# wdmwhh/MRefSR

Hardware: AMD Instinct MI355X
Metric: 4x SR Mpix/sec, 5-ref 160x160->640x640; PSNR within 0.01 dB of ref (higher is better)
Workload: dtype f32

## Files before the change

include/mrefsr_hip.h:

```cpp
#ifndef MREFSR_HIP_H
#define MREFSR_HIP_H

#include <stdint.h>

#ifdef __cplusplus
extern "C" {
#endif

#define MREFSR_ABI_VERSION 1

enum {
    MREFSR_OK = 0,
    MREFSR_E_INVALID = -1,
    MREFSR_E_UNSUPPORTED = -2,
    MREFSR_E_LAUNCH = -3
};

typedef void *mrefsr_stream_t;

int mrefsr_abi_version(void);
const char *mrefsr_last_error(void);


int mrefsr_corr_padded_channels(int C);
// ... 71 lines not shown
int mrefsr_conv_wgrad1x1_f32(const float *g, const float *x, const float *g_amax, float *grad_weight, void *workspace,
                             int64_t workspace_bytes, int64_t pixels, int Cout, int ld_g, int Cin, int ld_x, int *range_flag,
                             mrefsr_stream_t stream);
int mrefsr_dcn_fwd(const void *x, const void *offset, const void *mask, const void *weight, const void *bias,
                   void *out, const mrefsr_dcn_shape *s, float act_slope, int dtype, mrefsr_stream_t stream);
int mrefsr_dcn_im2col(const void *x, const void *offset, const void *mask, void *columns,
                      const mrefsr_dcn_shape *s, int dtype, mrefsr_stream_t stream);
int mrefsr_dcn_col2im(const void *grad_col, const void *x, const void *offset, const void *mask, void *grad_x,
                      void *grad_offset, void *grad_mask, const mrefsr_dcn_shape *s, int dtype,
                      mrefsr_stream_t stream);


int mrefsr_mrattn_fwd_f32(const float *q, const float *emb, const float *ass, float *out,
                          float *prob, int N, int T, int c, int c2, int HW, int t_major,
                          mrefsr_stream_t stream);
int mrefsr_mrattn_fwd_nhwc_f32(const float *q, const float *emb, const float *ass, float *out, int N,
                               int T, int c, int HW, mrefsr_stream_t stream);
int mrefsr_mrattn_fwd_nhwc_scaled_f32(const float *q, const float *emb, const float *ass, float *out, int N,
                                      int T, int c, int HW, float q_scale, mrefsr_stream_t stream);
int mrefsr_mrattn_bwd_f32(const float *q, const float *emb, const float *ass, const float *prob,
                          const float *g_out, float *g_q, float *g_emb, float *g_ass, int N,
                          int T, int c, int c2, int HW, int t_major, mrefsr_stream_t stream);
int mrefsr_mrattn_fwd_nhwc_bf16(const void *q, const void *emb, const void *ass, void *out, int N, int T,
                                int c, int HW, mrefsr_stream_t stream);
int mrefsr_mrattn_fwd_masked_f32(const float *q, const float *emb, const float *ass, const uint32_t *valid_bits, float *out,
                                 float *prob, int N, int T, int c, int c2, int HW, int t_major, mrefsr_stream_t stream);
int mrefsr_mrattn_bwd_masked_f32(const float *q, const float *emb, const float *ass, const float *prob, const float *g_out,
                                 const uint32_t *valid_bits, float *g_q, float *g_emb, float *g_ass, int N, int T, int c, int c2,
                                 int HW, int t_major, mrefsr_stream_t stream);
int mrefsr_mrattn_fwd_nhwc_masked_f32(const float *q, const float *emb, const float *ass, const uint32_t *valid_bits, float *out,
                                      int N, int T, int c, int HW, float q_scale, mrefsr_stream_t stream);
int mrefsr_mrattn_fwd_nhwc_masked_bf16(const void *q, const void *emb, const void *ass, const uint32_t *valid_bits, void *out, int N,
                                       int T, int c, int HW, mrefsr_stream_t stream);


int mrefsr_fused_bias_act(const void *x, const void *bias, const void *ref, void *out,
                          int64_t size_x, int step_b, int size_b, int act, int grad, float alpha,
                          float scale, int dtype, mrefsr_stream_t stream);

int mrefsr_tail_bilinear_add_f32(const float *y_nhwc, const float *x, float *out, int B, int C, int h, int w, int scale, int ld,
                                 mrefsr_stream_t stream);

int mrefsr_bias_act_res_f32(const float *x, const float *bias, const float *pre, int64_t pre_N,
                            const float *residual, float *out, int64_t N, int C, int64_t HW,
                            float slope, mrefsr_stream_t stream);

typedef struct mrefsr_conv_desc {
    int32_t N, H, W, ksize;
    int32_t C1, ld1, N1;
    int32_t C2, ld2, N2;
    int32_t Cout, ld_out, ld_res, pre_N;
    int32_t act, epilogue, terms;
    float slope;
    float wscale;
} mrefsr_conv_desc;
int64_t mrefsr_conv_packed_bytes(int Cout, int Cin, int ksize, int terms);
int mrefsr_conv_pack_weight_f32(const float *weight, void *packed, int Cout, int Cin, int ksize, int terms,
                                float wscale, mrefsr_stream_t stream);
int mrefsr_conv_pack_weight_view_f32(const float *weight, void *packed, int Cout, int Cin, int ksize, int terms, float wscale,
                                     int64_t stride_o, int64_t stride_i, int flip, mrefsr_stream_t stream);
typedef struct mrefsr_conv_pack_job {
    const float *weight;
    void *packed;
    int64_t stride_o, stride_i;
    int32_t Cout, Cin, ksize, terms, flip;
    float wscale;
// ... 328 lines not shown
```

mrefsr_amd/_lib.py:

```python
import ctypes as C
import os

_HERE = os.path.dirname(os.path.abspath(__file__))
LIB_PATH = os.environ.get('MREFSR_HIP_LIB') or os.path.join(_HERE, 'lib', 'libmrefsr_hip.so')
ABI_VERSION = 1

_vp, _i, _f, _i64 = C.c_void_p, C.c_int, C.c_float, C.c_int64


class DcnShape(C.Structure):
    _fields_ = [(n, C.c_int) for n in ('B', 'C', 'H', 'W', 'Co', 'kh', 'kw', 'stride_h', 'stride_w', 'pad_h', 'pad_w',
                                       'dil_h', 'dil_w', 'groups', 'dg')]


class ConvDesc(C.Structure):
    _fields_ = [(n, C.c_int32) for n in ('N', 'H', 'W', 'ksize', 'C1', 'ld1', 'N1', 'C2', 'ld2', 'N2', 'Cout', 'ld_out', 'ld_res',
                                         'pre_N', 'act', 'epilogue', 'terms')] + [('slope', C.c_float), ('wscale', C.c_float)]


class ConvPackJob(C.Structure):
    _fields_ = [('weight', C.c_void_p), ('packed', C.c_void_p), ('stride_o', C.c_int64), ('stride_i', C.c_int64), ('Cout', C.c_int32),
                ('Cin', C.c_int32), ('ksize', C.c_int32), ('terms', C.c_int32), ('flip', C.c_int32), ('wscale', C.c_float)]


# ... 26 lines not shown
    'mrefsr_pixnorm_f32': (_i, [_vp, _vp, _vp, _vp, _i, _i, _i, _i, _i, _i, _vp, _vp]),
    'mrefsr_patch_norm_f32': (_i, [_vp, _vp, _vp, _i, _i, _i, _vp]),
    'mrefsr_corr_top1_f32': (_i, [_vp, _vp, _vp, _vp, _vp, _vp, _i, _i, _i, _i, _i, _vp]),
    'mrefsr_feature_match_index_workspace_bytes': (_i64, [_i, _i, _i, _i]),
    'mrefsr_feature_match_index_f32': (_i, [_vp, _vp] + [_i] * 10 + [_vp, _vp, _vp, _i64, _vp]),
    'mrefsr_corr_workspace_bytes': (_i64, [_i, _i, _i]),
    'mrefsr_corr_prefilter_info': (_i64, [_i, _i, _i, _i, C.c_char_p, _i, C.POINTER(C.c_int)]),
    'mrefsr_corr_top1_prefilter_f32': (_i, [_vp] * 9 + [_i64, _i, _i, _i, _i, _i, _i, _vp, _vp]),
    'mrefsr_offsets_from_idx_f32': (_i, [_vp, _vp, _vp, _vp, _i, _i, _i, _vp]),
    'mrefsr_dynagg_prep_f32': (_i, [_vp, _vp, _vp, _vp, _vp, _vp, _i, _i, _i, _i, _i, _vp]),
    'mrefsr_dynagg_prep_bwd_f32': (_i, [_vp, _vp, _vp, _vp, _i, _i, _i, _i, _vp]),
    'mrefsr_dynagg_prep_bwd_nhwc_f32': (_i, [_vp, _vp, _vp, _vp, _vp, _vp, _i, _i, _i, _i, _vp]),
    'mrefsr_dynagg_prep_bwd_blocks': (_i, [_i, _i, _i, _i]),
    'mrefsr_dynagg_prep_bwd_det_workspace_bytes': (_i64, [_i, _i, _i, _i]),
    'mrefsr_dynagg_prep_bwd_nhwc_det_f32': (_i, [_vp, _vp, _vp, _vp, _vp, _vp, _i, _i, _i, _i, _vp, _i64, _vp, _vp]),
    'mrefsr_dcn_fwd_workspace_bytes': (_i64, [C.POINTER(DcnShape)]),
    'mrefsr_dcn_fwd_f32': (_i, [_vp, _vp, _vp, _vp, _vp, _vp, C.POINTER(DcnShape), _f, _i, _vp, _i64, _vp, _vp]),
    'mrefsr_dcn_fwd_amax_f32': (_i, [_vp, _vp, _vp, _vp, _vp, _vp, C.POINTER(DcnShape), _f, _i, _vp, _i64, _vp, _vp, _vp]),
    'mrefsr_dcn_im2col_f32': (_i, [_vp, _vp, _vp, _vp, C.POINTER(DcnShape), _vp]),
    'mrefsr_dcn_col2im_f32': (_i, [_vp, _vp, _vp, _vp, _vp, _vp, _vp, C.POINTER(DcnShape), _vp]),
    'mrefsr_dcn_bwd_data_f32': (_i, [_vp, _vp, _vp, _vp, _vp, _f, _vp, _vp, _vp, _vp, C.POINTER(DcnShape), _vp]),
    'mrefsr_dcn_bwd_weight_workspace_bytes': (_i64, [C.POINTER(DcnShape)]),
    'mrefsr_conv_wgrad1x1_workspace_bytes': (_i64, [_i64, _i, _i]),
    'mrefsr_conv_wgrad1x1_f32': (_i, [_vp, _vp, _vp, _vp, _vp, _i64, _i64, _i, _i, _i, _i, _vp, _vp]),
    'mrefsr_dcn_bwd_weight_f32': (_i, [_vp, _vp, _vp, _vp, _vp, _vp, _vp, _i64, C.POINTER(DcnShape), _vp, _vp]),
    'mrefsr_mrattn_fwd_f32': (_i, [_vp, _vp, _vp, _vp, _vp, _i, _i, _i, _i, _i, _i, _vp]),
    'mrefsr_mrattn_fwd_nhwc_f32': (_i, [_vp, _vp, _vp, _vp, _i, _i, _i, _i, _vp]),
    'mrefsr_mrattn_fwd_nhwc_scaled_f32': (_i, [_vp, _vp, _vp, _vp, _i, _i, _i, _i, _f, _vp]),
    'mrefsr_mrattn_bwd_f32': (_i, [_vp, _vp, _vp, _vp, _vp, _vp, _vp, _vp, _i, _i, _i, _i, _i, _i, _vp]),
    'mrefsr_mrattn_fwd_masked_f32': (_i, [_vp] * 6 + [_i] * 6 + [_vp]),
    'mrefsr_mrattn_bwd_masked_f32': (_i, [_vp] * 9 + [_i] * 6 + [_vp]),
    'mrefsr_mrattn_fwd_nhwc_masked_f32': (_i, [_vp] * 5 + [_i, _i, _i, _i, _f, _vp]),
    'mrefsr_mrattn_fwd_nhwc_masked_bf16': (_i, [_vp] * 5 + [_i, _i, _i, _i, _vp]),
    'mrefsr_fused_bias_act': (_i, [_vp, _vp, _vp, _vp, _i64, _i, _i, _i, _i, _f, _f, _i, _vp]),
    'mrefsr_bias_act_res_f32': (_i, [_vp, _vp, _vp, _i64, _vp, _vp, _i64, _i, _i64, _f, _vp]),
    'mrefsr_tail_bilinear_add_f32': (_i, [_vp, _vp, _vp, _i, _i, _i, _i, _i, _i, _vp]),
    'mrefsr_conv_packed_bytes': (_i64, [_i, _i, _i, _i]),
    'mrefsr_conv_pack_weight_f32': (_i, [_vp, _vp, _i, _i, _i, _i, _f, _vp]),
    'mrefsr_conv_pack_weight_view_f32': (_i, [_vp, _vp, _i, _i, _i, _i, _f, _i64, _i64, _i, _vp]),
    'mrefsr_conv_pack_weights_multi_f32': (_i, [_vp, _i, _vp, _vp]),
    'mrefsr_act_bwd_blocks': (_i, [_i64, _i]),
    'mrefsr_act_bwd_nhwc_f32': (_i, [_vp, _vp, _vp, _i, _vp, _vp, _vp, _i64, _i, _i, _f, _vp, _vp, _vp]),
    'mrefsr_act_bwd_det_workspace_bytes': (_i64, [_i64, _i]),
    'mrefsr_act_bwd_nhwc_det_f32': (_i, [_vp, _vp, _vp, _i, _vp, _vp, _vp, _i64, _i, _i, _f, _vp, _vp, _vp, _i64, _vp, _vp]),
    'mrefsr_conv_nhwc_scaled_f32': (_i, [C.POINTER(ConvDesc), _vp, _vp, _vp, _vp, _vp, _vp, _vp, _vp, _vp, _vp, _vp]),
    'mrefsr_conv_nhwc_amax_f32': (_i, [C.POINTER(ConvDesc), _vp, _vp, _vp, _vp, _vp, _vp, _vp, _vp, _vp, _vp, _vp, _vp]),
    'mrefsr_conv_nhwc_bwd_f32': (_i, [C.POINTER(ConvDesc), _vp, _vp, _vp, _i, _vp, _vp, _vp, _vp, _vp, _vp]),
    'mrefsr_conv_nhwc_bwd_det_workspace_bytes': (_i64, [C.POINTER(ConvDesc)]),
    'mrefsr_conv_nhwc_bwd_det_f32': (_i, [C.POINTER(ConvDesc), _vp, _vp, _vp, _i, _vp, _vp, _vp, _vp, _vp, _vp, _i64, _vp, _vp]),
    'mrefsr_conv_wgrad3x3_workspace_bytes': (_i64, [_i, _i, _i, _i, _i]),
    'mrefsr_conv_wgrad3x3_f32': (_i, [_vp, _i, _i, _vp, _i, _i, _vp, _i64, _i64, _i, _vp, _i, _i, _i, _vp, _i64, _vp, _vp]),
    'mrefsr_conv_wgrad3x3_batch_workspace_bytes': (_i64, [_i, _i, _i, _i, _i, _i]),
    'mrefsr_conv_wgrad3x3_batch_f32': (_i, [_i, _vp, _i, _i, _vp, _i, _i, _vp, _i64, _i64, _i, _vp, _i, _i, _i, _vp, _i64, _vp, _vp]),
    'mrefsr_mrattn_bwd_nhwc_f32': (_i, [_vp, _vp, _vp, _vp, _vp, _vp, _vp, _i, _i, _i, _i, _vp]),
    'mrefsr_mrattn_bwd_nhwc_masked_f32': (_i, [_vp] * 8 + [_i, _i, _i, _i, _vp]),
    'mrefsr_attn_modulate_bwd_f32': (_i, [_vp, _vp, _vp, _vp, _vp, _i64, _vp]),
    'mrefsr_reflect_pad_nhwc_f32': (_i, [_vp, _vp] + [_i] * 6 + [_vp]),
    'mrefsr_reflect_pad_bwd_nhwc_f32': (_i, [_vp, _vp] + [_i] * 6 + [_vp]),
    'mrefsr_crop_nhwc_f32': (_i, [_vp, _vp, _vp] + [_i] * 6 + [_vp]),
    'mrefsr_crop_bwd_nhwc_f32': (_i, [_vp, _vp] + [_i] * 6 + [_vp]),
    'mrefsr_conv_nhwc_f32': (_i, [C.POINTER(ConvDesc), _vp, _vp, _vp, _vp, _vp, _vp, _vp, _vp, _vp, _vp]),
    'mrefsr_dcn_fwd': (_i, [_vp, _vp, _vp, _vp, _vp, _vp, C.POINTER(DcnShape), _f, _i, _vp]),
    'mrefsr_dcn_im2col': (_i, [_vp, _vp, _vp, _vp, C.POINTER(DcnShape), _i, _vp]),
    'mrefsr_dcn_col2im': (_i, [_vp, _vp, _vp, _vp, _vp, _vp, _vp, C.POINTER(DcnShape), _i, _vp]),
    'mrefsr_conv_dynagg_f32': (_i, [C.POINTER(ConvDesc), _vp, _vp, _vp, _vp, _vp, _vp, _vp, _i, _vp, _vp]),
    'mrefsr_mrattn_fwd_nhwc_bf16': (_i, [_vp, _vp, _vp, _vp, _i, _i, _i, _i, _vp]),
# ... 180 lines not shown
```

mrefsr_amd/archs/ref_mrapa_restoration_arch.py:

```python
import logging

import torch
import torch.nn as nn
import torch.nn.functional as F
from torch.autograd import Function
from torch.autograd.function import once_differentiable

from .. import hip
from ..ops.dcn import modulated_deform_conv
from ..utils.registry import ARCH_REGISTRY
from . import nhwc, nhwc_train
from .arch_util import ResidualBlockNoBN, conv_act, default_init_weights, make_layer, ref_valid_bits, srntt_init_weights


class _DynAggPrep(Function):

    @staticmethod
    def forward(ctx, om, pre_offset, dg, abs_sum, om_bias=None):
        om = om.contiguous()
        offset, mask = hip.dynagg_prep(om, pre_offset.contiguous(), dg, abs_sum, om_bias)
        ctx.dg = dg
        ctx.save_for_backward(mask)
        return offset, mask

# ... 296 lines not shown
        return all((4 - s % 4) % 4 < s for side in (h, w) for s in (side, 2 * side))

    def spatial_padding(self, feats):
        _, _, h, w = feats.size()
        pad_h, pad_w = self.pads(h, w)
        if pad_h == 0 and pad_w == 0:
            return feats
        return F.pad(feats, [0, pad_w, 0, pad_h], mode='reflect')

    def forward(self, target, refs, ref_valid=None):
        t = len(refs)
        return self._fuse(target, torch.stack(refs, dim=1).flatten(0, 1), t, t_major=False, ref_valid=ref_valid)

    def forward_stacked(self, target, refs, t, ref_valid=None):
        return self._fuse(target, refs, t, t_major=True, ref_valid=ref_valid)

    def forward_nhwc(self, target, refs, t, ref_valid=None):
        h_in, w_in = target.shape[1:3]
        ph, pw = self.pads(h_in, w_in)
        vb = ref_valid_bits(ref_valid, target.shape[0], t, target.device)
        if ph or pw:
            if target.dtype != torch.float32:
                target = nhwc.to_nhwc(self.spatial_padding(nhwc.as_nchw(target)))
                refs = nhwc.to_nhwc(self.spatial_padding(nhwc.as_nchw(refs)))
                return self.forward_nhwc(target, refs, t, vb)[:, :h_in, :w_in, :].contiguous()
            out = self.forward_nhwc(nhwc.reflect_pad(target, ph, pw), nhwc.reflect_pad(refs, ph, pw), t, vb)
            return nhwc.crop(out, h_in, w_in)
        q = nhwc.conv(self.conv_emb1[0], target, prelu=self.conv_emb1[1], amax=False)
        train = q.requires_grad
        fold = not train and q.dtype == torch.float32 and not nhwc.BF16
        if not fold:
            q = q * self.scale if train else nhwc.rnd_(q.mul_(self.scale))
        emb = nhwc.conv(self.conv_emb2[0], refs, prelu=self.conv_emb2[1], amax=False)
        ass = nhwc.conv(self.conv_ass, refs, amax=False)
        if vb is not None:
            if fold:
                r = hip.mrattn_fwd_nhwc_masked(q, emb, ass, t, vb, q_scale=float(self.scale))
            else:
                r = nhwc_train.attention(q, emb, ass, t, vb) if train else nhwc.rnd_(hip.mrattn_fwd_nhwc_masked(q, emb, ass, t, vb))
        elif fold:
            r = hip.mrattn_fwd_nhwc(q, emb, ass, t, q_scale=float(self.scale))
        else:
            r = nhwc_train.attention(q, emb, ass, t) if train else nhwc.rnd_(hip.mrattn_fwd_nhwc(q, emb, ass, t))
        del emb, ass
        attn = nhwc.conv(self.spatial_attn, target, x2=r, slope=0.1)
        attn_mul = nhwc.conv(self.spatial_attn_mul2, nhwc.conv(self.spatial_attn_mul1, attn, slope=0.1), amax=False)
        attn_add = nhwc.conv(self.spatial_attn_add2, nhwc.conv(self.spatial_attn_add1, attn, slope=0.1), amax=False)
        r = nhwc_train.modulate(r, attn_mul, attn_add) if train else nhwc.rnd_(hip.attn_modulate_(r, attn_mul, attn_add))
        return nhwc.conv(self.feat_fusion, target, x2=r, slope=0.1)

    def _fuse(self, target, refs, t, t_major, ref_valid=None):
        h_input, w_input = target.shape[-2:]
        vb = ref_valid_bits(ref_valid, target.shape[0], t, target.device)
        target = self.spatial_padding(target)
        refs = self.spatial_padding(refs)
        q = self.conv_emb1(target) * self.scale
        emb = self.conv_emb2(refs)
        ass = conv_act(self.conv_ass, refs)
        refs = _MultiRefAttention.apply(q, emb, ass, t, t_major) if vb is None else _MultiRefAttention.apply(q, emb, ass, t, t_major, vb)
        attn = conv_act(self.spatial_attn, torch.cat([target, refs], dim=1), 0.1)
        attn_mul = conv_act(self.spatial_attn_mul2, conv_act(self.spatial_attn_mul1, attn, 0.1))
        attn_add = conv_act(self.spatial_attn_add2, conv_act(self.spatial_attn_add1, attn, 0.1))
        attn_mul = torch.sigmoid(attn_mul)
        refs = refs * attn_mul * 2 + attn_add
        feat = conv_act(self.feat_fusion, torch.cat([target, refs], dim=1), 0.1)
        if feat.shape[-2:] != (h_input, w_input):
            feat = feat[:, :, :h_input, :w_input].contiguous()
        return feat
```

mrefsr_amd/csrc/mrattn.hip:

```cpp
#include "common.h"

namespace {

constexpr int MAX_T = 16;

template <bool MASKED> __device__ __forceinline__ bool on(unsigned int bits, int t) { return !MASKED || ((bits >> t) & 1u); }

template <bool MASKED>
__global__ __launch_bounds__(256) void mrattn_fwd_kernel(const float *__restrict__ q, const float *__restrict__ emb,
                                                         const float *__restrict__ ass, float *__restrict__ out,
                                                         float *__restrict__ prob, int N, int T, int c, int c2, int HW, int t_major,
                                                         const unsigned int *__restrict__ valid_bits)
{
    const long total = (long)N * HW;
    for (long e = blockIdx.x * (long)blockDim.x + threadIdx.x; e < total; e += (long)gridDim.x * blockDim.x) {
        const int n = (int)(e / HW), p = (int)(e - (long)n * HW);
        const unsigned int vb = MASKED ? valid_bits[n] : 0u;
        float s[MAX_T];
#pragma unroll
        for (int t = 0; t < MAX_T; ++t) s[t] = 0.f;
        const size_t i0 = t_major ? (size_t)n : (size_t)n * T, is = t_major ? (size_t)N : 1;
        const float *qp = q + (size_t)n * c * HW + p;
        const float *ep = emb + i0 * c * HW + p;
        const size_t est = is * c * HW;
// ... 162 lines not shown
                }
#pragma unroll
                for (int o = L / 2; o > 0; o >>= 1) d += __shfl_xor(d, o, 64);
                logit[t] = d;
                if (on<MASKED>(vb, t)) mx = fmaxf(mx, d);
            }
        }
        float den = 0.f;
#pragma unroll
        for (int t = 0; t < 16; ++t)
            if (t < T && on<MASKED>(vb, t)) {
                logit[t] = expf(logit[t] - mx);
                den += logit[t];
            }
        const float inv = (!MASKED || den > 0.f) ? 1.0f / den : 0.f;
        float4 o0 = make_float4(0.f, 0.f, 0.f, 0.f), o1 = o0;
#pragma unroll
        for (int t = 0; t < 16; ++t)
            if (t < T && on<MASKED>(vb, t)) {
                const float w = logit[t] * inv;
                const typename IO::T *ap = ass + (((long)t * N + n) * HW + p) * (2 * CH) + 4 * sub;
                const float4 a0 = IO::ld(ap), a1 = IO::ld(ap + CH);
                o0.x += w * a0.x, o0.y += w * a0.y, o0.z += w * a0.z, o0.w += w * a0.w;
                o1.x += w * a1.x, o1.y += w * a1.y, o1.z += w * a1.z, o1.w += w * a1.w;
            }
        if (ok) {
            typename IO::T *op = out + g * (2 * CH) + 4 * sub;
            IO::st(op, o0);
            IO::st(op + CH, o1);
        }
    }
}

template <bool IO16, bool MASKED>
int launch_mrattn_nhwc(const void *q, const void *emb, const void *ass, const unsigned int *vb, void *out, int N, int T, int c, int HW, float q_scale,
                       hipStream_t st)
{
    typedef typename Io4<IO16>::T E;
    const long waves = ((long)N * HW * (c / 4) + 63) / 64;
    const long blocks = (waves + 3) / 4;
    const dim3 grid((int)(blocks < 65536 ? blocks : 65536));
    const E *q_ = (const E *)q, *e_ = (const E *)emb, *a_ = (const E *)ass;
    E *o_ = (E *)out;
    if (c == 256) hipLaunchKernelGGL((mrattn_fwd_nhwc_kernel<256, IO16, MASKED>), grid, dim3(256), 0, st, q_, e_, a_, o_, N, T, (long)HW, q_scale, vb);
    else if (c == 128) hipLaunchKernelGGL((mrattn_fwd_nhwc_kernel<128, IO16, MASKED>), grid, dim3(256), 0, st, q_, e_, a_, o_, N, T, (long)HW, q_scale, vb);
    else if (c == 64) hipLaunchKernelGGL((mrattn_fwd_nhwc_kernel<64, IO16, MASKED>), grid, dim3(256), 0, st, q_, e_, a_, o_, N, T, (long)HW, q_scale, vb);
    else return mrefsr::fail(MREFSR_E_UNSUPPORTED, "mrattn_fwd_nhwc: c=%d (64, 128 or 256: the three MRAPAFusion heads)", c);
    return mrefsr::check_launch("mrattn_fwd_nhwc");
}

}

MREFSR_EXPORT int mrefsr_mrattn_fwd_nhwc_f32(const float *q, const float *emb, const float *ass, float *out, int N, int T, int c,
                                             int HW, mrefsr_stream_t stream)
{
    MREFSR_REQUIRE(q && emb && ass && out, "mrattn_fwd_nhwc: null pointer");
    MREFSR_REQUIRE(N > 0 && T > 0 && T <= 16 && HW > 0, "mrattn_fwd_nhwc: N=%d T=%d HW=%d (T <= 16)", N, T, HW);
    return launch_mrattn_nhwc<false, false>(q, emb, ass, nullptr, out, N, T, c, HW, 1.0f, (hipStream_t)stream);
}

MREFSR_EXPORT int mrefsr_mrattn_fwd_nhwc_scaled_f32(const float *q, const float *emb, const float *ass, float *out, int N, int T, int c,
                                                    int HW, float q_scale, mrefsr_stream_t stream)
{
    MREFSR_REQUIRE(q && emb && ass && out, "mrattn_fwd_nhwc_scaled: null pointer");
    MREFSR_REQUIRE(N > 0 && T > 0 && T <= 16 && HW > 0, "mrattn_fwd_nhwc_scaled: N=%d T=%d HW=%d (T <= 16)", N, T, HW);
    return launch_mrattn_nhwc<false, false>(q, emb, ass, nullptr, out, N, T, c, HW, q_scale, (hipStream_t)stream);
}

MREFSR_EXPORT int mrefsr_mrattn_fwd_nhwc_bf16(const void *q, const void *emb, const void *ass, void *out, int N, int T, int c, int HW,
                                              mrefsr_stream_t stream)
{
    MREFSR_REQUIRE(q && emb && ass && out, "mrattn_fwd_nhwc_bf16: null pointer");
    MREFSR_REQUIRE(N > 0 && T > 0 && T <= 16 && HW > 0, "mrattn_fwd_nhwc_bf16: N=%d T=%d HW=%d (T <= 16)", N, T, HW);
    return launch_mrattn_nhwc<true, false>(q, emb, ass, nullptr, out, N, T, c, HW, 1.0f, (hipStream_t)stream);
}

MREFSR_EXPORT int mrefsr_mrattn_fwd_f32(const float *q, const float *emb, const float *ass, float *out, float *prob,
                                        int N, int T, int c, int c2, int HW, int t_major, mrefsr_stream_t stream)
{
    MREFSR_REQUIRE(q && emb && ass && out, "mrattn_fwd: null pointer");
    if (int e = check("mrattn_fwd", N, T, c, c2, HW)) return e;
    const long blocks = ((long)N * HW + 255) / 256;
    hipLaunchKernelGGL(mrattn_fwd_kernel<false>, dim3((int)(blocks < 65536 ? blocks : 65536)), dim3(256), 0, (hipStream_t)stream,
                       q, emb, ass, out, prob, N, T, c, c2, HW, t_major, (const unsigned int *)nullptr);
    return mrefsr::check_launch("mrattn_fwd");
}

MREFSR_EXPORT int mrefsr_mrattn_bwd_f32(const float *q, const float *emb, const float *ass, const float *prob,
                                        const float *g_out, float *g_q, float *g_emb, float *g_ass, int N, int T, int c,
                                        int c2, int HW, int t_major, mrefsr_stream_t stream)
{
    MREFSR_REQUIRE(q && emb && ass && prob && g_out && g_q && g_emb && g_ass, "mrattn_bwd: null pointer");
    if (int e = check("mrattn_bwd", N, T, c, c2, HW)) return e;
    const long blocks = ((long)N * HW + 255) / 256;
    hipLaunchKernelGGL(mrattn_bwd_kernel<false>, dim3((int)(blocks < 65536 ? blocks : 65536)), dim3(256), 0, (hipStream_t)stream,
                       q, emb, ass, prob, g_out, g_q, g_emb, g_ass, N, T, c, c2, HW, t_major, (const unsigned int *)nullptr);
    return mrefsr::check_launch("mrattn_bwd");
}

MREFSR_EXPORT int mrefsr_mrattn_fwd_nhwc_masked_f32(const float *q, const float *emb, const float *ass, const uint32_t *valid_bits, float *out,
                                                    int N, int T, int c, int HW, float q_scale, mrefsr_stream_t stream)
// ... 41 lines not shown
```

mrefsr_amd/hip.py:

```python
import contextlib
import ctypes as C
import math

import torch

from . import _lib
from .param_cache import Packed as _Packed, param_stamp
from ._lib import DcnShape


def _stream():
    return C.c_void_p(torch.cuda.current_stream().cuda_stream)


_timing = {'on': False, 'detail': False, 'events': {}, 'work': {}}


def set_kernel_timing(on=True, detail=False):
    _timing['on'] = bool(on)
    _timing['detail'] = bool(on and detail)
    _timing['events'] = {}
    _timing['work'] = {}
    _timing['bytes'] = {}

# ... 535 lines not shown
        raise ValueError(f'{name}: valid_bits must be an int32 tensor of shape ({n},)')


def mrattn_fwd_masked(q, emb, ass, t, valid_bits, want_prob=True, t_major=False):
    _chk('mrattn_fwd_masked', q, emb, ass)
    n, c, h, w = q.shape
    c2 = ass.shape[1]
    if emb.shape[0] != n * t or ass.shape[0] != n * t or emb.shape[1] != c:
        raise ValueError('mrattn_fwd_masked: inconsistent shapes')
    _chk_valid_bits('mrattn_fwd_masked', valid_bits, n)
    out = torch.empty((n, c2, h, w), device=q.device, dtype=torch.float32)
    prob = torch.empty((n, t, h, w), device=q.device, dtype=torch.float32) if want_prob else None
    _lib.call('mrefsr_mrattn_fwd_masked_f32', _p(q), _p(emb), _p(ass), _p(valid_bits), _p(out), _p(prob), n, t, c, c2, h * w,
              1 if t_major else 0, _stream())
    return out, prob


def mrattn_fwd_nhwc_masked(q, emb, ass, t, valid_bits, q_scale=None):
    b16 = q.dtype == torch.bfloat16
    if q_scale is not None and b16:
        raise TypeError('mrattn_fwd_nhwc_masked: q_scale goes with fp32 tensors')
    _chk('mrattn_fwd_nhwc_masked', q, emb, ass, dtype=q.dtype if b16 else torch.float32)
    n, h, w, c = q.shape
    if tuple(emb.shape) != (n * t, h, w, c) or tuple(ass.shape) != (n * t, h, w, 2 * c):
        raise ValueError('mrattn_fwd_nhwc_masked: inconsistent shapes')
    _chk_valid_bits('mrattn_fwd_nhwc_masked', valid_bits, n)
    out = torch.empty((n, h, w, 2 * c), device=q.device, dtype=q.dtype)
    with _timed('mrattn_fwd', (3.0 * t + 3.0) * c * h * w * q.element_size() * n, detail=True):
        if b16:
            _lib.call('mrefsr_mrattn_fwd_nhwc_masked_bf16', _p(q), _p(emb), _p(ass), _p(valid_bits), _p(out), n, t, c, h * w, _stream())
        else:
            _lib.call('mrefsr_mrattn_fwd_nhwc_masked_f32', _p(q), _p(emb), _p(ass), _p(valid_bits), _p(out), n, t, c, h * w,
                      C.c_float(1.0 if q_scale is None else q_scale), _stream())
    return out


def mrattn_bwd_masked(q, emb, ass, prob, g_out, t, valid_bits, t_major=False, out=None):
    _chk('mrattn_bwd_masked', q, emb, ass, prob, g_out)
    n, c, h, w = q.shape
    c2 = ass.shape[1]
    if (emb.shape[0] != n * t or ass.shape[0] != n * t or emb.shape[1] != c or tuple(prob.shape) != (n, t, h, w)
            or tuple(g_out.shape) != (n, c2, h, w)):
        raise ValueError('mrattn_bwd_masked: inconsistent shapes')
    _chk_valid_bits('mrattn_bwd_masked', valid_bits, n)
    g_q, g_emb, g_ass = _grad_triple('mrattn_bwd_masked', out, q, emb, ass)
    _lib.call('mrefsr_mrattn_bwd_masked_f32', _p(q), _p(emb), _p(ass), _p(prob), _p(g_out), _p(valid_bits), _p(g_q), _p(g_emb), _p(g_ass),
              n, t, c, c2, h * w, 1 if t_major else 0, _stream())
    return g_q, g_emb, g_ass


def _grad_triple(name, out, q, emb, ass):
    if out is None:
        return torch.empty_like(q), torch.empty_like(emb), torch.empty_like(ass)
    _chk(name, *out)
    if [tuple(o.shape) for o in out] != [tuple(v.shape) for v in (q, emb, ass)]:
        raise ValueError(f'{name}: out must be (g_q, g_emb, g_ass) shaped like (q, emb, ass)')
    return tuple(out)


_DT = {torch.float32: 0, torch.float16: 1, torch.bfloat16: 2, torch.float64: 3}


def fused_bias_act(x, bias, ref, act, grad, alpha, scale):
    if x.dtype not in _DT:
        raise TypeError(f'fused_bias_act: unsupported dtype {x.dtype}')
    x = x.contiguous()
# ... 1933 lines not shown
```

Measured before the change: 16.86.

## Blend reference features by attention before the assoc conv instead of after

Because the value convolution is linear, the attention-weighted sum over T references can be taken before the 3x3 conv_ass instead of after it. A new kernel computes only the softmax probabilities from q and emb, and a second fused kernel blends the refs per pixel in LDS and runs a single C->2C 3x3 MFMA conv with split-f16 precision. The bias term is scaled by the probability sum. This replaces T convolutions plus an attention kernel with one conv, which cuts FLOPs and removes the large ass intermediate. In exchange the rounding order differs and a custom conv path must hold PSNR.

Result: faster. 17.45, median of 6 (+3.5%).

```diff
diff --git a/include/mrefsr_hip.h b/include/mrefsr_hip.h
--- a/include/mrefsr_hip.h
+++ b/include/mrefsr_hip.h
@@ -127,6 +127,11 @@
                                       int N, int T, int c, int HW, float q_scale, mrefsr_stream_t stream);
 int mrefsr_mrattn_fwd_nhwc_masked_bf16(const void *q, const void *emb, const void *ass, const uint32_t *valid_bits, void *out, int N,
                                        int T, int c, int HW, mrefsr_stream_t stream);
+int mrefsr_mrattn_prob_nhwc_f32(const float *q, const float *emb, const uint32_t *valid_bits, float *prob, int N, int T, int c,
+                                int HW, float q_scale, mrefsr_stream_t stream);
+int mrefsr_mrattn_blend_conv_f32(const float *refs, const float *prob, const void *packed, const float *bias, const uint32_t *valid_bits,
+                                 const float *in_amax, int *range_flag, float *out, int N, int T, int H, int W, int C, float wscale,
+                                 mrefsr_stream_t stream);
 
 
 int mrefsr_fused_bias_act(const void *x, const void *bias, const void *ref, void *out,
diff --git a/mrefsr_amd/_lib.py b/mrefsr_amd/_lib.py
--- a/mrefsr_amd/_lib.py
+++ b/mrefsr_amd/_lib.py
@@ -82,6 +82,8 @@
     'mrefsr_mrattn_bwd_masked_f32': (_i, [_vp] * 9 + [_i] * 6 + [_vp]),
     'mrefsr_mrattn_fwd_nhwc_masked_f32': (_i, [_vp] * 5 + [_i, _i, _i, _i, _f, _vp]),
     'mrefsr_mrattn_fwd_nhwc_masked_bf16': (_i, [_vp] * 5 + [_i, _i, _i, _i, _vp]),
+    'mrefsr_mrattn_prob_nhwc_f32': (_i, [_vp] * 4 + [_i, _i, _i, _i, _f, _vp]),
+    'mrefsr_mrattn_blend_conv_f32': (_i, [_vp] * 8 + [_i, _i, _i, _i, _i, _f, _vp]),
     'mrefsr_fused_bias_act': (_i, [_vp, _vp, _vp, _vp, _i64, _i, _i, _i, _i, _f, _f, _i, _vp]),
     'mrefsr_bias_act_res_f32': (_i, [_vp, _vp, _vp, _i64, _vp, _vp, _i64, _i, _i64, _f, _vp]),
     'mrefsr_tail_bilinear_add_f32': (_i, [_vp, _vp, _vp, _i, _i, _i, _i, _i, _i, _vp]),
diff --git a/mrefsr_amd/archs/ref_mrapa_restoration_arch.py b/mrefsr_amd/archs/ref_mrapa_restoration_arch.py
--- a/mrefsr_amd/archs/ref_mrapa_restoration_arch.py
+++ b/mrefsr_amd/archs/ref_mrapa_restoration_arch.py
@@ -352,6 +352,14 @@
         if not fold:
             q = q * self.scale if train else nhwc.rnd_(q.mul_(self.scale))
         emb = nhwc.conv(self.conv_emb2[0], refs, prelu=self.conv_emb2[1], amax=False)
+        if self.blend_first(fold, refs, t):
+            prob = hip.mrattn_prob_nhwc(q, emb, t, vb, q_scale=float(self.scale))
+            del emb
+            r = hip.mrattn_blend_conv(refs, prob, hip.packed_weight(self.conv_ass.weight, None, 16),
+                                      None if self.conv_ass.bias is None else self.conv_ass.bias.detach(), t, vb,
+                                      in_amax=nhwc.amax_of(refs) if nhwc.WINO_INSCALE else None)
+            del prob
+            return self._modulate_fuse(target, r, train)
         ass = nhwc.conv(self.conv_ass, refs, amax=False)
         if vb is not None:
             if fold:
@@ -363,6 +371,15 @@
         else:
             r = nhwc_train.attention(q, emb, ass, t) if train else nhwc.rnd_(hip.mrattn_fwd_nhwc(q, emb, ass, t))
         del emb, ass
+        return self._modulate_fuse(target, r, train)
+
+    BLEND_FIRST = True
+
+    def blend_first(self, fold, refs, t):
+        return (self.BLEND_FIRST and fold and nhwc.TERMS == 16 and not hip.is_range_free() and refs.dtype == torch.float32
+                and refs.shape[3] in (64, 128, 256) and self.conv_ass.out_channels == 2 * refs.shape[3] and t <= 16)
+
+    def _modulate_fuse(self, target, r, train):
         attn = nhwc.conv(self.spatial_attn, target, x2=r, slope=0.1)
         attn_mul = nhwc.conv(self.spatial_attn_mul2, nhwc.conv(self.spatial_attn_mul1, attn, slope=0.1), amax=False)
         attn_add = nhwc.conv(self.spatial_attn_add2, nhwc.conv(self.spatial_attn_add1, attn, slope=0.1), amax=False)
diff --git a/mrefsr_amd/csrc/mrattn.hip b/mrefsr_amd/csrc/mrattn.hip
--- a/mrefsr_amd/csrc/mrattn.hip
+++ b/mrefsr_amd/csrc/mrattn.hip
@@ -218,6 +218,68 @@
     }
 }
 
+template <int CH, bool MASKED>
+__global__ __launch_bounds__(256) void mrattn_prob_nhwc_kernel(const float *__restrict__ q, const float *__restrict__ emb, float *__restrict__ prob,
+                                                               int N, int T, long HW, float q_scale, const unsigned int *__restrict__ valid_bits)
+{
+    typedef Io4<false> IO;
+    constexpr int L = CH / 4, PPW = 64 / L;
+    const int lane = threadIdx.x & 63, sub = lane % L, pw = lane / L;
+    const long total = (long)N * HW;
+    const long wave = (blockIdx.x * (long)blockDim.x + threadIdx.x) >> 6, nwave = ((long)gridDim.x * blockDim.x) >> 6;
+    for (long base = wave * PPW; base < total; base += nwave * PPW) {
+        const long gp = base + pw;
+        const bool ok = gp < total;
+        const long g = ok ? gp : total - 1;
+        const long n = g / HW, p = g - n * HW;
+        const unsigned int vb = MASKED ? valid_bits[n] : 0u;
+        float4 qv = IO::ld(q + g * CH + 4 * sub);
+        qv.x *= q_scale, qv.y *= q_scale, qv.z *= q_scale, qv.w *= q_scale;
+        float logit[16];
+        float mx = -3.4e38f;
+#pragma unroll
+        for (int t = 0; t < 16; ++t) {
+            if (t < T) {
+                float d = 0.f;
+                if (on<MASKED>(vb, t)) {
+                    const float4 e = IO::ld(emb + (((long)t * N + n) * HW + p) * CH + 4 * sub);
+                    d = qv.x * e.x + qv.y * e.y + qv.z * e.z + qv.w * e.w;
+                }
+#pragma unroll
+                for (int o = L / 2; o > 0; o >>= 1) d += __shfl_xor(d, o, 64);
+                logit[t] = d;
+                if (on<MASKED>(vb, t)) mx = fmaxf(mx, d);
+            }
+        }
+        float den = 0.f;
+#pragma unroll
+        for (int t = 0; t < 16; ++t)
+            if (t < T && on<MASKED>(vb, t)) {
+                logit[t] = expf(logit[t] - mx);
+                den += logit[t];
+            }
+        const float inv = (!MASKED || den > 0.f) ? 1.0f / den : 0.f;
+        float mine = 0.f;
+#pragma unroll
+        for (int t = 0; t < 16; ++t)
+            if (t < T && sub == t) mine = on<MASKED>(vb, t) ? logit[t] * inv : 0.f;
+        if (ok && sub < T) prob[g * T + sub] = mine;
+    }
+}
+
+template <bool MASKED>
+int launch_mrattn_prob(const float *q, const float *emb, const unsigned int *vb, float *prob, int N, int T, int c, int HW, float q_scale, hipStream_t st)
+{
+    const long waves = ((long)N * HW * (c / 4) + 63) / 64;
+    const long blocks = (waves + 3) / 4;
+    const dim3 grid((int)(blocks < 65536 ? blocks : 65536));
+    if (c == 256) hipLaunchKernelGGL((mrattn_prob_nhwc_kernel<256, MASKED>), grid, dim3(256), 0, st, q, emb, prob, N, T, (long)HW, q_scale, vb);
+    else if (c == 128) hipLaunchKernelGGL((mrattn_prob_nhwc_kernel<128, MASKED>), grid, dim3(256), 0, st, q, emb, prob, N, T, (long)HW, q_scale, vb);
+    else if (c == 64) hipLaunchKernelGGL((mrattn_prob_nhwc_kernel<64, MASKED>), grid, dim3(256), 0, st, q, emb, prob, N, T, (long)HW, q_scale, vb);
+    else return mrefsr::fail(MREFSR_E_UNSUPPORTED, "mrattn_prob_nhwc: c=%d (64, 128 or 256: the three MRAPAFusion heads)", c);
+    return mrefsr::check_launch("mrattn_prob_nhwc");
+}
+
 template <bool IO16, bool MASKED>
 int launch_mrattn_nhwc(const void *q, const void *emb, const void *ass, const unsigned int *vb, void *out, int N, int T, int c, int HW, float q_scale,
                        hipStream_t st)
@@ -253,6 +315,15 @@
     return launch_mrattn_nhwc<false, false>(q, emb, ass, nullptr, out, N, T, c, HW, q_scale, (hipStream_t)stream);
 }
 
+MREFSR_EXPORT int mrefsr_mrattn_prob_nhwc_f32(const float *q, const float *emb, const uint32_t *valid_bits, float *prob, int N, int T, int c,
+                                              int HW, float q_scale, mrefsr_stream_t stream)
+{
+    MREFSR_REQUIRE(q && emb && prob, "mrattn_prob_nhwc: null pointer");
+    MREFSR_REQUIRE(N > 0 && T > 0 && T <= 16 && HW > 0, "mrattn_prob_nhwc: N=%d T=%d HW=%d (T <= 16)", N, T, HW);
+    return valid_bits ? launch_mrattn_prob<true>(q, emb, valid_bits, prob, N, T, c, HW, q_scale, (hipStream_t)stream)
+                      : launch_mrattn_prob<false>(q, emb, nullptr, prob, N, T, c, HW, q_scale, (hipStream_t)stream);
+}
+
 MREFSR_EXPORT int mrefsr_mrattn_fwd_nhwc_bf16(const void *q, const void *emb, const void *ass, void *out, int N, int T, int c, int HW,
                                               mrefsr_stream_t stream)
 {
diff --git a/mrefsr_amd/csrc/mrattn_conv.hip b/mrefsr_amd/csrc/mrattn_conv.hip
--- /dev/null
+++ b/mrefsr_amd/csrc/mrattn_conv.hip
@@ -0,0 +1,259 @@
+#include "conv_common.h"
+
+namespace {
+using namespace mrefsr_conv;
+
+constexpr int TG = 5;
+constexpr int TR = 8, TW = 32;
+constexpr int PH = TR + 2, PW = TW + 2, NPIX = PH * PW;
+constexpr int QPL = NPIX * 16;
+constexpr int TPL = 4 * QPL;
+constexpr int NPIECE = NPIX * 4;
+constexpr int NPK = (NPIECE + 255) / 256;
+constexpr int NJ = 4;
+constexpr int LDS_RAW = TG * TPL;
+constexpr int LDS_BYTES = LDS_RAW + TR * TW * 4 + 64 + 16;
+
+struct BlendArgs {
+    const float *refs, *prob, *bias, *in_amax;
+    const unsigned short *wp;
+    const unsigned int *valid_bits;
+    int *range_flag;
+    float *out;
+    int N, T, H, W, ncb;
+    float out_scale;
+};
+
+template <int C, bool MASKED>
+__global__ __launch_bounds__(256) void mrattn_blend_conv_kernel(const BlendArgs A)
+{
+    constexpr int NCH = C / KC, COUT = 2 * C, TAPS = 9, NW = 3;
+    extern __shared__ __align__(16) unsigned char smem[];
+    float *psum = reinterpret_cast<float *>(smem + LDS_RAW);
+    int *tlist = reinterpret_cast<int *>(smem + LDS_RAW + TR * TW * 4);
+    const int tid = threadIdx.x, lane = tid & 63, wv = tid >> 6, l31 = lane & 31, kh = lane >> 5;
+    const int H = A.H, W = A.W, T = A.T, N = A.N;
+    const int tx_n = (W + TW - 1) / TW, ty_n = (H + TR - 1) / TR;
+    const unsigned int lin = blockIdx.x, seq = lin >> 3;
+    const int cbk = (int)(seq % (unsigned)A.ncb);
+    const long tile = (long)(seq / (unsigned)A.ncb) * 8 + (lin & 7u);
+    if (tile >= (long)tx_n * ty_n * N) return;
+    const int n = (int)(tile / (tx_n * ty_n)), trem = (int)(tile - (long)n * (tx_n * ty_n));
+    const int y0 = (trem / tx_n) * TR, x0 = (trem % tx_n) * TW;
+
+    if (tid == 0) {
+        const unsigned int vb = MASKED ? A.valid_bits[n] : 0xffffffffu;
+        int c = 0;
+        for (int t = 0; t < T; ++t)
+            if ((vb >> t) & 1u) tlist[c++] = t;
+        tlist[16] = c;
+    }
+    float in_s = 1.f, oscale = A.out_scale;
+    if (A.in_amax) {
+        const float am = *A.in_amax;
+        if (am > 1.0e-30f && am < 3.0e38f) {
+            int e;
+            (void)frexpf(am, &e);
+            in_s = ldexpf(1.f, 14 - e);
+            oscale = A.out_scale * ldexpf(1.f, e - 14);
+        }
+    }
+    __syncthreads();
+    const int total = __builtin_amdgcn_readfirstlane(tlist[16]);
+    const int n_grp = (total + TG - 1) / TG, n_it = NCH * n_grp;
+
+    const float *prow[2];
+    bool pok[2];
+#pragma unroll
+    for (int m = 0; m < 2; ++m) {
+        const int gy = y0 + wv * 2 + m, gx = x0 + l31;
+        pok[m] = gy < H && gx < W;
+        prow[m] = A.prob + (((size_t)n * H + (gy < H ? gy : H - 1)) * W + (gx < W ? gx : W - 1)) * T;
+        float s = 0.f;
+        for (int k = 0; k < total; ++k) s += prow[m][__builtin_amdgcn_readfirstlane(tlist[k])];
+        if (kh == 0) psum[(wv * 2 + m) * TW + l31] = pok[m] ? s : 0.f;
+    }
+
+    f32x16 acc[2][NJ];
+#pragma unroll
+    for (int m = 0; m < 2; ++m)
+#pragma unroll
+        for (int j = 0; j < NJ; ++j)
+#pragma unroll
+            for (int e = 0; e < 16; ++e) acc[m][j][e] = 0.f;
+
+    int goff[NPK], loff[NPK];
+    unsigned int in_map = 0u, in_tile = 0u;
+#pragma unroll
+    for (int k = 0; k < NPK; ++k) {
+        const int i = tid + k * 256;
+        const int p = i >> 2, q = i & 3;
+        const int py = p / PW, px = p - py * PW;
+        const int gy = y0 + py - 1, gx = x0 + px - 1;
+        const bool tile = i < NPIECE, ok = tile && gy >= 0 && gy < H && gx >= 0 && gx < W;
+        goff[k] = ok ? (gy * W + gx) * C + 4 * q : 0;
+        loff[k] = q * QPL + p * 16;
+        in_map |= (ok ? 1u : 0u) << k, in_tile |= (tile ? 1u : 0u) << k;
+    }
+    float4 pf[TG][NPK];
+    auto fetch = [&](const int it) {
+        const int ch = it / n_grp, g = it - ch * n_grp;
+        const int cnt = total - g * TG < TG ? total - g * TG : TG;
+#pragma unroll
+        for (int tg = 0; tg < TG; ++tg)
+            if (tg < cnt) {
+                const int t = __builtin_amdgcn_readfirstlane(tlist[g * TG + tg]);
+                const float *base = A.refs + ((size_t)t * N + n) * H * W * C + ch * KC;
+#pragma unroll
+                for (int k = 0; k < NPK; ++k)
+                    pf[tg][k] = ((in_map >> k) & 1u) ? *reinterpret_cast<const float4 *>(base + goff[k]) : make_float4(0.f, 0.f, 0.f, 0.f);
+            }
+    };
+    if (n_it) fetch(0);
+
+    const unsigned short *wlane = A.wp + (size_t)l31 * KC + kh * 8;
+    auto bload = [&](const int lin, u32x4 (&b)[NJ][2]) {
+#pragma unroll
+        for (int j = 0; j < NJ; ++j)
+#pragma unroll
+            for (int sp = 0; sp < 2; ++sp)
+                b[j][sp] = *reinterpret_cast<const u32x4 *>(wlane + ((((size_t)(cbk * 2 + (j >> 1)) * NCH * TAPS + lin) * NW + sp) * NB + (j & 1) * 32) * KC);
+    };
+
+    bool bad = false;
+    float pr[2][TG];
+    for (int it = 0; it < n_it; ++it) {
+        const int ch = it / n_grp, g = it - ch * n_grp;
+        const int cnt = total - g * TG < TG ? total - g * TG : TG;
+        if (it) __syncthreads();
+#pragma unroll
+        for (int tg = 0; tg < TG; ++tg)
+            if (tg < cnt) {
+#pragma unroll
+                for (int k = 0; k < NPK; ++k) {
+                    float4 v = pf[tg][k];
+                    v.x *= in_s, v.y *= in_s, v.z *= in_s, v.w *= in_s;
+                    bad = bad || !(fmaxf(fmaxf(fabsf(v.x), fabsf(v.y)), fmaxf(fabsf(v.z), fabsf(v.w))) <= 65000.f);
+                    if ((in_tile >> k) & 1u) *reinterpret_cast<float4 *>(smem + tg * TPL + loff[k]) = v;
+                }
+            }
+        __syncthreads();
+        if (it + 1 < n_it) fetch(it + 1);
+        if (n_grp > 1 || it == 0) {
+#pragma unroll
+            for (int m = 0; m < 2; ++m)
+#pragma unroll
+                for (int k = 0; k < TG; ++k) pr[m][k] = (k < cnt && pok[m]) ? prow[m][__builtin_amdgcn_readfirstlane(tlist[g * TG + k])] : 0.f;
+        }
+        u32x4 b[NJ][2];
+        bload(ch * TAPS, b);
+#pragma nounroll
+        for (int tap = 0; tap < TAPS; ++tap) {
+            const int dy = (tap * 11) >> 5, dx = tap - 3 * dy;
+            u32x4 bn[NJ][2];
+            if (tap + 1 < TAPS) bload(ch * TAPS + tap + 1, bn);
+#pragma unroll
+            for (int m = 0; m < 2; ++m) {
+                const unsigned char *sp = smem + (2 * kh) * QPL + ((wv * 2 + m + dy) * PW + l31 + dx) * 16;
+                float u[8];
+#pragma unroll
+                for (int c = 0; c < 8; ++c) u[c] = 0.f;
+#pragma unroll
+                for (int k = 0; k < TG; ++k)
+                    if (k < cnt) {
+                        const float4 s0 = *reinterpret_cast<const float4 *>(sp + k * TPL);
+                        const float4 s1 = *reinterpret_cast<const float4 *>(sp + k * TPL + QPL);
+                        const float w = pr[m][k];
+                        u[0] = fmaf(w, s0.x, u[0]), u[1] = fmaf(w, s0.y, u[1]), u[2] = fmaf(w, s0.z, u[2]), u[3] = fmaf(w, s0.w, u[3]);
+                        u[4] = fmaf(w, s1.x, u[4]), u[5] = fmaf(w, s1.y, u[5]), u[6] = fmaf(w, s1.z, u[6]), u[7] = fmaf(w, s1.w, u[7]);
+                    }
+                u32x4 ah, al;
+#pragma unroll
+                for (int c = 0; c < 4; ++c) {
+                    ah[c] = pk_f16(u[2 * c], u[2 * c + 1]);
+                    const f32x2 h = un_f16(ah[c]);
+                    al[c] = pk_f16((u[2 * c] - h[0]) * 2048.f, (u[2 * c + 1] - h[1]) * 2048.f);
+                }
+#pragma unroll
+                for (int j = 0; j < NJ; ++j)
+                    acc[m][j] = __builtin_amdgcn_mfma_f32_32x32x16_f16(__builtin_bit_cast(f16x8, ah), __builtin_bit_cast(f16x8, b[j][1]), acc[m][j], 0, 0, 0);
+#pragma unroll
+                for (int j = 0; j < NJ; ++j)
+                    acc[m][j] = __builtin_amdgcn_mfma_f32_32x32x16_f16(__builtin_bit_cast(f16x8, al), __builtin_bit_cast(f16x8, scale_wh(b[j][0])), acc[m][j], 0, 0, 0);
+#pragma unroll
+                for (int j = 0; j < NJ; ++j)
+                    acc[m][j] = __builtin_amdgcn_mfma_f32_32x32x16_f16(__builtin_bit_cast(f16x8, ah), __builtin_bit_cast(f16x8, b[j][0]), acc[m][j], 0, 0, 0);
+            }
+            if (tap + 1 < TAPS) {
+#pragma unroll
+                for (int j = 0; j < NJ; ++j) b[j][0] = bn[j][0], b[j][1] = bn[j][1];
+            }
+        }
+    }
+    if (bad && A.range_flag) atomicOr(A.range_flag, 1);
+    __syncthreads();
+
+#pragma unroll
+    for (int m = 0; m < 2; ++m) {
+        const int gy = y0 + wv * 2 + m;
+        if (gy >= H) continue;
+#pragma unroll
+        for (int j = 0; j < NJ; ++j) {
+            const int co = cbk * (NJ * 32) + j * 32 + l31;
+            const float bv = A.bias ? A.bias[co] : 0.f;
+            float *orow = A.out + (((size_t)n * H + gy) * W) * COUT + co;
+#pragma unroll
+            for (int e = 0; e < 16; ++e) {
+                const int x = (e & 3) + 8 * (e >> 2) + 4 * kh, gx = x0 + x;
+                if (gx < W) orow[(size_t)gx * COUT] = acc[m][j][e] * oscale + bv * psum[(wv * 2 + m) * TW + x];
+            }
+        }
+    }
+}
+
+template <int C, bool MASKED> int launch_blend_c(const BlendArgs &a, const dim3 grid, hipStream_t st)
+{
+    static unsigned long long attr_done = 0;
+    if (mrefsr::first_use_on_device(attr_done)) {
+        const hipError_t e = hipFuncSetAttribute(reinterpret_cast<const void *>(&mrattn_blend_conv_kernel<C, MASKED>),
+                                                 hipFuncAttributeMaxDynamicSharedMemorySize, LDS_BYTES);
+        if (e != hipSuccess) {
+            attr_done = 0;
+            (void)hipGetLastError();
+            return mrefsr::fail(MREFSR_E_LAUNCH, "mrattn_blend_conv: %d bytes of dynamic LDS refused: %s", LDS_BYTES, hipGetErrorString(e));
+        }
+    }
+    hipLaunchKernelGGL((mrattn_blend_conv_kernel<C, MASKED>), grid, dim3(256), LDS_BYTES, st, a);
+    return mrefsr::check_launch("mrattn_blend_conv");
+}
+
+template <bool MASKED> int launch_blend(const BlendArgs &a, int C, hipStream_t st)
+{
+    const long tiles = (long)((a.W + TW - 1) / TW) * ((a.H + TR - 1) / TR) * a.N;
+    const dim3 grid((unsigned)(((tiles + 7) / 8) * 8 * a.ncb));
+    if (C == 64) return launch_blend_c<64, MASKED>(a, grid, st);
+    if (C == 128) return launch_blend_c<128, MASKED>(a, grid, st);
+    return launch_blend_c<256, MASKED>(a, grid, st);
+}
+
+}
+
+MREFSR_EXPORT int mrefsr_mrattn_blend_conv_f32(const float *refs, const float *prob, const void *packed, const float *bias,
+                                               const uint32_t *valid_bits, const float *in_amax, int *range_flag, float *out, int N, int T,
+                                               int H, int W, int C, float wscale, mrefsr_stream_t stream)
+{
+    MREFSR_REQUIRE(refs && prob && packed && out, "mrattn_blend_conv: null pointer");
+    MREFSR_REQUIRE(N > 0 && T > 0 && T <= 16 && H > 0 && W > 0, "mrattn_blend_conv: N=%d T=%d H=%d W=%d (T <= 16)", N, T, H, W);
+    MREFSR_REQUIRE((int64_t)((W + TW - 1) / TW) * ((H + TR - 1) / TR) * N < (int64_t)1 << 28, "mrattn_blend_conv: N=%d H=%d W=%d (too many tiles)", N, H, W);
+    MREFSR_REQUIRE((int64_t)H * W * 256 < (int64_t)1 << 31, "mrattn_blend_conv: H=%d W=%d (32-bit offsets inside a map)", H, W);
+    MREFSR_REQUIRE(wscale > 0.f, "mrattn_blend_conv: wscale=%g", (double)wscale);
+    if (C != 64 && C != 128 && C != 256)
+        return mrefsr::fail(MREFSR_E_UNSUPPORTED, "mrattn_blend_conv: c=%d (64, 128 or 256: the three MRAPAFusion heads)", C);
+    BlendArgs a;
+    a.refs = refs, a.prob = prob, a.bias = bias, a.in_amax = in_amax;
+    a.wp = reinterpret_cast<const unsigned short *>(packed);
+    a.valid_bits = valid_bits, a.range_flag = range_flag, a.out = out;
+    a.N = N, a.T = T, a.H = H, a.W = W, a.ncb = 2 * C / (NJ * 32);
+    a.out_scale = 1.0f / wscale;
+    return valid_bits ? launch_blend<true>(a, C, (hipStream_t)stream) : launch_blend<false>(a, C, (hipStream_t)stream);
+}
diff --git a/mrefsr_amd/hip.py b/mrefsr_amd/hip.py
--- a/mrefsr_amd/hip.py
+++ b/mrefsr_amd/hip.py
@@ -591,6 +591,39 @@
         else:
             _lib.call('mrefsr_mrattn_fwd_nhwc_masked_f32', _p(q), _p(emb), _p(ass), _p(valid_bits), _p(out), n, t, c, h * w,
                       C.c_float(1.0 if q_scale is None else q_scale), _stream())
+    return out
+
+
+def mrattn_prob_nhwc(q, emb, t, valid_bits=None, q_scale=1.0):
+    _chk('mrattn_prob_nhwc', q, emb)
+    n, h, w, c = q.shape
+    if tuple(emb.shape) != (n * t, h, w, c):
+        raise ValueError('mrattn_prob_nhwc: inconsistent shapes')
+    if valid_bits is not None:
+        _chk_valid_bits('mrattn_prob_nhwc', valid_bits, n)
+    prob = torch.empty((n, h, w, t), device=q.device, dtype=torch.float32)
+    with _timed('mrattn_prob', ((t + 1.0) * c + t) * h * w * 4.0 * n, detail=True):
+        _lib.call('mrefsr_mrattn_prob_nhwc_f32', _p(q), _p(emb), _p(valid_bits), _p(prob), n, t, c, h * w, C.c_float(q_scale), _stream())
+    return prob
+
+
+def mrattn_blend_conv(refs, prob, packed, bias, t, valid_bits=None, in_amax=None):
+    _chk('mrattn_blend_conv', refs, prob, bias, in_amax)
+    if packed.terms != 16:
+        raise ValueError('mrattn_blend_conv: weights packed with terms=16 expected')
+    tn, h, w, c = refs.shape
+    n = prob.shape[0]
+    if tn != n * t or tuple(prob.shape) != (n, h, w, t):
+        raise ValueError('mrattn_blend_conv: inconsistent shapes')
+    if packed.data.numel() != _lib.load().mrefsr_conv_packed_bytes(2 * c, c, 3, 16) or (bias is not None and bias.numel() != 2 * c):
+        raise ValueError('mrattn_blend_conv: weight / bias do not belong to a C -> 2C 3x3 convolution')
+    if valid_bits is not None:
+        _chk_valid_bits('mrattn_blend_conv', valid_bits, n)
+    out = torch.empty((n, h, w, 2 * c), device=refs.device, dtype=torch.float32)
+    nby = (refs.numel() + prob.numel() + out.numel()) * 4.0 + 4.0 * c * 2 * c * 9
+    with _timed('mrattn_blend_conv', 2.0 * n * h * w * c * 2 * c * 9, detail=True, nbytes=nby):
+        _lib.call('mrefsr_mrattn_blend_conv_f32', _p(refs), _p(prob), _p(packed.data), _p(bias), _p(valid_bits), _p(in_amax),
+                  _p(_range_flag(refs.device)), _p(out), n, t, h, w, c, C.c_float(packed.wscale), _stream())
     return out
 
 
```
